# SteveMacenski/slam_toolbox

Measured on NVIDIA H100. Metric: scan matches/sec (1081-beam, +-2m/+-20deg), higher is better.
Workload: dtype u8

## Files before the change

### include/b200slam.h

```cpp
#ifndef B200SLAM_H
#define B200SLAM_H

#include <stdint.h>

#ifdef __cplusplus
extern "C" {
#endif

#define B200_OK 0
#define B200_ERR_INVALID_ARG 1
#define B200_ERR_CUDA 2
#define B200_ERR_UNSUPPORTED 3
#define B200_ERR_NOT_FOUND 4
#define B200_ERR_NUMERIC 5

const char * b200_last_error(void);
int b200_set_device(int ordinal);
int b200_device_count(void);
void b200_parallel_for(int32_t n, void (*fn)(int32_t, void *), void * ctx);
int32_t b200_host_threads(void);


typedef struct b200sm_params {
  double search_size;
// ... 51 lines not shown
                        const int32_t * pair_query, const int32_t * pair_chain, int32_t npairs,
                        int32_t do_penalize);
int b200sm_batch_run(b200sm * h);
int b200sm_batch_fetch(b200sm * h, double * response, double * mean, double * cov);
int b200sm_batch_kernel_ms(b200sm * h, float * ms);
int b200sm_batch_best(b200sm * h, int32_t * best_sum, int32_t * best_index, int32_t * tie_count);
int b200sm_batch_reduce_keys(b200sm * h, void * device_keys, int64_t id_offset);
int32_t b200sm_batch_winner_record_bytes(void);
int b200sm_batch_winner_records(b200sm * h, void * device_records, int64_t id_offset);
int b200sm_batch_winners_select(b200sm * h, const void * device_gathered, int32_t nranks, int64_t * winner_id,
                                double * response, double * mean, double * cov);
int b200sm_batch_info(b200sm * h, int32_t info[8]);
int b200sm_batch_tile_info(b200sm * h, int32_t info[8]);
int b200sm_batch_tile_layout(b200sm * h, int32_t layout[4]);
int b200sm_batch_tile_stats(b200sm * h, int32_t stats[8]);
int b200sm_batch_fetch_stats(b200sm * h, int32_t stats[4]);
int b200sm_batch_upload_timing(b200sm * h, double out[3]);
int b200sm_batch_transfer_bytes(b200sm * h, int64_t * h2d_bytes, int64_t * d2h_bytes, int32_t reset);
int b200sm_set_option(b200sm * h, const char * name, int32_t value);
int b200sm_match_timing(b200sm * h, double out[6], int32_t reset);
int64_t b200sm_launch_count(const b200sm * h);


typedef struct b200pg_opts {
  int32_t max_num_iterations;
  double function_tolerance;
  double gradient_tolerance;
  double parameter_tolerance;
  double min_relative_decrease;
  double initial_trust_region_radius;
// ... 98 lines not shown
```

### slam_toolbox_b200/api.py

```python
from __future__ import annotations

import ctypes as C
import math
import os
from dataclasses import dataclass

import numpy as np

from . import build as _build

_DP = C.POINTER(C.c_double)
_IP = C.POINTER(C.c_int32)
_lib = None

OK, ERR_INVALID_ARG, ERR_CUDA, ERR_UNSUPPORTED, ERR_NOT_FOUND, ERR_NUMERIC = range(6)


class B200Error(RuntimeError):
    def __init__(self, code: int, msg: str):
        super().__init__(f"b200slam error {code}: {msg}")
        self.code = code


class SmParams(C.Structure):
# ... 63 lines not shown
    L.b200sm_grid_copy.argtypes = [C.c_void_p, C.POINTER(C.c_uint8), C.c_int32]
    L.b200sm_match_batch.argtypes = [C.c_void_p, C.POINTER(CScan), C.c_int32, C.POINTER(CScan), C.c_int32, _IP, C.c_int32,
                                     _IP, _IP, C.c_int32, C.c_int32, C.c_int32, _DP, _DP, _DP]
    L.b200sm_batch_upload.argtypes = [C.c_void_p, C.POINTER(CScan), C.c_int32, C.POINTER(CScan), C.c_int32, _IP, C.c_int32,
                                      _IP, _IP, C.c_int32, C.c_int32]
    L.b200sm_batch_run.argtypes = [C.c_void_p]
    L.b200sm_batch_fetch.argtypes = [C.c_void_p, _DP, _DP, _DP]
    L.b200sm_batch_kernel_ms.argtypes = [C.c_void_p, C.POINTER(C.c_float)]
    L.b200sm_batch_best.argtypes = [C.c_void_p, _IP, _IP, _IP]
    L.b200sm_batch_info.argtypes = [C.c_void_p, _IP]
    L.b200sm_batch_winner_record_bytes.restype = C.c_int32
    L.b200sm_batch_winner_records.argtypes = [C.c_void_p, C.c_void_p, C.c_int64]
    L.b200sm_batch_winners_select.argtypes = [C.c_void_p, C.c_void_p, C.c_int32, C.POINTER(C.c_int64), _DP, _DP, _DP]
    L.b200sm_batch_tile_info.argtypes = [C.c_void_p, _IP]
    L.b200sm_batch_tile_stats.argtypes = [C.c_void_p, _IP]
    L.b200sm_batch_tile_layout.argtypes = [C.c_void_p, _IP]
    L.b200sm_batch_fetch_stats.argtypes = [C.c_void_p, _IP]
    L.b200sm_batch_upload_timing.argtypes = [C.c_void_p, _DP]
    L.b200sm_batch_reduce_keys.argtypes = [C.c_void_p, C.c_void_p, C.c_int64]
    L.b200sm_batch_transfer_bytes.argtypes = [C.c_void_p, C.POINTER(C.c_int64), C.POINTER(C.c_int64), C.c_int32]
    L.b200sm_set_option.argtypes = [C.c_void_p, C.c_char_p, C.c_int32]
    L.b200sm_match_timing.argtypes = [C.c_void_p, _DP, C.c_int32]
    L.b200sm_launch_count.restype = C.c_int64
    L.b200sm_launch_count.argtypes = [C.c_void_p]
    if hasattr(L, "b200pg_create"):
        L.b200pg_default_opts.argtypes = [C.POINTER(PgOpts)]
        L.b200pg_create.argtypes = [C.POINTER(PgOpts), C.POINTER(C.c_void_p)]
        L.b200pg_destroy.argtypes = [C.c_void_p]
        L.b200pg_set_stream.argtypes = [C.c_void_p, C.c_void_p]
        L.b200pg_reset.argtypes = [C.c_void_p]
# ... 244 lines not shown
    def batch_tile_info(self):
        info = np.zeros(8, dtype=np.int32)
        _check(lib().b200sm_batch_tile_info(self._h, _ip(info)))
        lay = np.zeros(4, dtype=np.int32)
        _check(lib().b200sm_batch_tile_layout(self._h, _ip(lay)))
        return dict(available=bool(info[0]), cluster=int(info[1]), chunks=int(info[2]), bands=int(info[3]), band_rows=int(info[4]),
                    refused_reason=int(info[5]), clusters=int(info[6]), smem_kb=int(info[7]), ytile_rows=int(lay[0]),
                    ytiles=int(lay[1]), xtiles=int(lay[2]), tail=bool(lay[3]))

    def batch_tile_stats(self):
        st = np.zeros(8, dtype=np.int32)
        _check(lib().b200sm_batch_tile_stats(self._h, _ip(st)))
        return dict(blocks=int(st[0]), sub_blocks=int(st[1]), max_edge_group=int(st[2]), split_groups=int(st[3]),
                    multi_entries=int(st[4]), max_multiplicity=int(st[5]), max_plain_group=int(st[6]), wrap2_entries=int(st[7]))

    def batch_upload_timing(self):
        t = np.zeros(3)
        _check(lib().b200sm_batch_upload_timing(self._h, _dp(t)))
        return dict(lookup_tables_ms=float(t[0]), kernel_tables_ms=float(t[1]), total_ms=float(t[2]))

    def batch_fetch_stats(self):
        st = np.zeros(4, dtype=np.int32)
        _check(lib().b200sm_batch_fetch_stats(self._h, _ip(st)))
        return dict(zero_pairs=int(st[0]), fallback_pairs=int(st[1]), pairs=int(st[2]))

    def transfer_bytes(self, reset: bool = False):
        a, b = C.c_int64(), C.c_int64()
        _check(lib().b200sm_batch_transfer_bytes(self._h, C.byref(a), C.byref(b), int(reset)))
        return a.value, b.value

# ... 223 lines not shown
```

### slam_toolbox_b200/csrc/sm_sweep.cu

```cuda
#include <algorithm>
#include <chrono>
#include <cmath>
#include <cstring>
#include <vector>

#include "common.cuh"
#include "sm_math.cuh"
#include "sm_types.cuh"
#include "sm_device.cuh"
#include "sm_sweep_dev.cuh"

namespace b200 {


constexpr int kFvWarps = 4;
constexpr int kFvBytesPerPoint = 17;
__global__ void __launch_bounds__(kFvWarps * 32) k_find_valid(SweepDev d)
{
  extern __shared__ __align__(16) unsigned char s_fv[];
  const int lane = threadIdx.x & 31, warp = threadIdx.x >> 5, nw = blockDim.x >> 5;
  const int item = blockIdx.x * nw + warp;
  if (item >= d.nitems) return;
  double2 * P = reinterpret_cast<double2 *>(s_fv) + (size_t)warp * d.max_n;
  unsigned char * valid = s_fv + (size_t)nw * d.max_n * sizeof(double2) + (size_t)warp * d.max_n;
// ... 1264 lines not shown
  if (!h) return B200_ERR_INVALID_ARG;
  return sweep_fetch(h, false, response, mean, cov);
  B200_GUARD_END
}

int b200sm_batch_kernel_ms(b200sm * h, float * ms)
{
  B200_GUARD_BEGIN
  if (!h || !ms || !h->sweep.ran) return B200_ERR_INVALID_ARG;
  B200_CUDA(cudaEventSynchronize(h->sweep.ev1));
  B200_CUDA(cudaEventElapsedTime(ms, h->sweep.ev0, h->sweep.ev1));
  return B200_OK;
  B200_GUARD_END
}

int b200sm_batch_best(b200sm * h, int32_t * best_sum, int32_t * best_index, int32_t * tie_count)
{
  B200_GUARD_BEGIN
  if (!h || !h->sweep.ran) return B200_ERR_INVALID_ARG;
  SweepHost & S = h->sweep;
  B200_CUDA(cudaMemcpyAsync(S.h_out.p, S.d_out.p, (size_t)S.npairs * sizeof(PairOut), cudaMemcpyDeviceToHost, h->stream));
  B200_CUDA(cudaStreamSynchronize(h->stream));
  for (int p = 0; p < S.npairs; ++p) {
    if (best_sum) best_sum[p] = S.h_out.p[p].best_sum;
    if (best_index) best_index[p] = S.h_out.p[p].tie_count > 0 ? S.h_out.p[p].ties[0] : -1;
    if (tie_count) tie_count[p] = S.h_out.p[p].tie_count;
  }
  return B200_OK;
  B200_GUARD_END
}
// ... 151 lines not shown
```

### slam_toolbox_b200/csrc/sm_tile.cu

```cuda
#include <algorithm>
#include <cmath>
#include <cstdlib>
#include <cstring>
#include <type_traits>
#include <vector>

#include "common.cuh"
#include "sm_math.cuh"
#include "sm_types.cuh"
#include "sm_device.cuh"
#include "sm_sweep_dev.cuh"

namespace b200 {

constexpr int kRowTiles = 6;
constexpr int kChunkBeams = 640;
constexpr int kMaxSingles = 63;
constexpr int kMaxPairs = 255;

__device__ __forceinline__ uint32_t smem_u32(const void * p) { return (uint32_t)__cvta_generic_to_shared(p); }
__device__ __forceinline__ void mbar_init(uint32_t bar, uint32_t count)
{
  asm volatile("mbarrier.init.shared::cta.b64 [%0], %1;" ::"r"(bar), "r"(count) : "memory");
}
// ... 81 lines not shown
    a.L2 = bL2 > a.L2 ? bL2 : a.L2;
  } else if (bL > a.L) {
    double l2 = a.L > a.L2 ? a.L : a.L2;
    l2 = bL2 > l2 ? bL2 : l2;
    a.L = bL; a.L2 = l2; a.cnt = bcnt; a.sum0 = bsum0;
    const int nb = bcnt < kMaxTies ? bcnt : kMaxTies;
    for (int t = 0; t < nb; ++t) a.ties[t] = bties[t];
  } else {
    double l2 = bL > a.L2 ? bL : a.L2;
    a.L2 = bL2 > l2 ? bL2 : l2;
  }
}

struct TileShared {
  unsigned long long bar[4];
  uint8_t kern[256];
  int ctr[2];
  double dscratch[32];
  int iscratch[32];
  TieRes chunk;
  TieRes res;
  double rankL[kTileMaxCluster], rankL2[kTileMaxCluster];
  int rankCnt[kTileMaxCluster], rankSum0[kTileMaxCluster];
  int rankTies[kTileMaxCluster][kMaxTies];
  double avg[2];
  double acc[4];
  int ok;
};

#ifdef B200_TILE_TIMERS
enum { kTmRaster, kTmDesc, kTmCorr, kTmFlush, kTmBarrier, kTmReduce, kTmPair, kTmTotal, kTmCount };
__device__ unsigned long long g_tile_timers[kTmCount];
#define TILE_TM_DECL                              \
  unsigned long long tm_acc[kTmCount] = {};       \
  long long tm_t = clock64();                     \
  const long long tm_start = tm_t;
#define TILE_TM(sec)                                                      \
  do {                                                                    \
    const long long tm_now = clock64();                                   \
    tm_acc[sec] += (unsigned long long)(tm_now - tm_t);                   \
    tm_t = tm_now;                                                        \
  } while (0)
#define TILE_TM_END                                                                 \
  do {                                                                              \
    TILE_TM(kTmPair);                                                               \
    tm_acc[kTmTotal] = (unsigned long long)(tm_t - tm_start);                       \
    if (lane == 0)                                                                  \
      for (int s = 0; s < kTmCount; ++s) atomicAdd(&g_tile_timers[s], tm_acc[s]);   \
  } while (0)
#else
#define TILE_TM_DECL
#define TILE_TM(sec) do {} while (0)
#define TILE_TM_END do {} while (0)
#endif

template <int kPitchW, bool kTail>
__global__ void __launch_bounds__(kTileThreads, 1) k_sweep_tile(SweepDev d, TileDev f)
{
  constexpr int kMain = kTail ? kRowTiles - 1 : kRowTiles;
  constexpr int kYTile = 8 * kMain;
  extern __shared__ __align__(128) unsigned char s_raw[];
  __shared__ TileShared sh;
  uint32_t * S = reinterpret_cast<uint32_t *>(s_raw);
  uint8_t * S8 = s_raw;
  int32_t * A = reinterpret_cast<int32_t *>(s_raw + f.off_A);
  double * probs = reinterpret_cast<double *>(s_raw + f.off_probs);
  int32_t * iprobs = reinterpret_cast<int32_t *>(s_raw + f.off_probs);
  const int C = f.C;
  const uint32_t rank = C > 1 ? cluster_rank() : 0u;
  const int cluster_id = blockIdx.x / C, nclusters = gridDim.x / C;
  const int nX = d.nX, nY = d.nY, nA = d.nA, P = nX * nY;
  const int half = d.ksize / 2, taps = d.ksize * d.ksize;
  const int tid = threadIdx.x, lane = tid & 31;
  const int y_l = lane >> 2, j_l = lane & 3;
  const int pitch_w = kPitchW ? kPitchW : f.pitch_w, pitchB = pitch_w * 4;
  const int sub_words = f.alloc_rows * pitch_w;
  const int nb = f.nbands;
  const uint32_t bar0 = smem_u32(&sh.bar[0]);
  const uint32_t stg0 = smem_u32(s_raw + f.off_stage);
  TILE_TM_DECL

  if (tid == 0) {
    mbar_init(bar0, 1);
    mbar_init(bar0 + 8, 1);
    mbar_init(bar0 + 16, 1);
    mbar_init(bar0 + 24, 1);
    asm volatile("fence.mbarrier_init.release.cluster;" ::: "memory");
    sh.ctr[0] = 0; sh.ctr[1] = 0;
  }
  const bool kern_smem = taps <= 256;
  if (kern_smem && tid < taps) sh.kern[tid] = d.kern[tid];
  const uint8_t * kern = kern_smem ? sh.kern : d.kern;
  __syncthreads();
  if (C > 1) { cluster_arrive(); cluster_wait(); }

  uint32_t cnt = 0;
  bool pending_wait = false;
  auto issue = [&](const TileSeq * e, uint32_t buf) {
    mbar_expect_tx(bar0 + 8 * buf, (uint32_t)e->bytes);
    bulk_g2s(stg0 + buf * (uint32_t)f.stage_bytes, f.desc + e->off, (uint32_t)e->bytes, bar0 + 8 * buf);
  };
  const uint32_t cel0 = smem_u32(s_raw + f.off_cells);
  const uint32_t cell_bytes = (uint32_t)f.cell_cap * 4u;
  auto issue_cells = [&](int pr, uint32_t buf) {
    const int it = min(d.pair_item_start[pr], max(d.nitems - 1, 0));
    mbar_expect_tx(bar0 + 16 + 8 * buf, cell_bytes);
    bulk_g2s(cel0 + buf * cell_bytes, d.cells + (size_t)it * d.max_n, cell_bytes, bar0 + 16 + 8 * buf);
  };
  if (cluster_id < d.npairs && tid == 0) {
    const int q0 = d.pair_query[cluster_id];
    issue(f.seq + f.seq_start[q0 * C + rank], 0);
    if (f.cell_cap) issue_cells(cluster_id, 0);
  }

  int iter = 0;
  for (int pair = cluster_id; pair < d.npairs; pair += nclusters, ++iter) {
    const int q = d.pair_query[pair];
    const uint32_t leader = (uint32_t)(iter % C);
    const TileSeq * seq = f.seq + f.seq_start[q * C + rank];
    const int nseq = f.seq_start[q * C + rank + 1] - f.seq_start[q * C + rank];
    const int it0 = d.pair_item_start[pair], it1 = d.pair_item_start[pair + 1];
    bool first_chunk = true;
    const int32_t * cells0 = d.cells + (size_t)it0 * d.max_n;
    const int ncell0 = it0 < it1 ? d.cell_count[it0] : 0;
    if (f.cell_cap) {
      if (tid == 0 && pair + nclusters < d.npairs) issue_cells(pair + nclusters, (uint32_t)((iter + 1) & 1));
      mbar_wait(bar0 + 16 + 8 * (iter & 1), (uint32_t)((iter >> 1) & 1));
      cells0 = reinterpret_cast<const int32_t *>(s_raw + f.off_cells + (size_t)(iter & 1) * cell_bytes);
    }
    TILE_TM(kTmPair);

    for (int si = 0; si < nseq; ++si) {
      const TileSeq e = seq[si];
      const int chunk_a0 = e.chunk * f.nAc;
      const int chunk_na = min(f.nAc, nA - chunk_a0);
      const int ph = e.stage / nb, band = e.stage - ph * nb;
      const int pp = ph & 1, pq = ph >> 1;
      const int band_r0 = band * f.band_rows;
      if (e.flags & kSeqNewChunk)
        for (int i = tid; i < chunk_na * P; i += kTileThreads) A[i] = 0;
      if (e.flags & kSeqNewStage) {
        {
          uint4 * S4 = reinterpret_cast<uint4 *>(s_raw);
          const uint4 zero = make_uint4(0u, 0u, 0u, 0u);
          for (int i = tid; i < (sub_words >> 2); i += kTileThreads) S4[i] = zero;
        }
        __syncthreads();
        const int nlev = f.nlevels;
        for (int lv = 0; lv < (nlev > 0 ? nlev : 1); ++lv) {
          const uint32_t want = nlev > 0 ? f.level[lv] : 0u;
          for (int it = it0; it < it1; ++it) {
            const int32_t * cl = it == it0 ? cells0 : d.cells + (size_t)it * d.max_n;
            const int ncell = it == it0 ? ncell0 : d.cell_count[it];
            for (int t = tid; t < ncell; t += kTileThreads) {
              const int32_t cell = cl[t];
              if (cell < 0) continue;
              const int cx = (cell & 0xFFFF) + d.roi_x - half, cy = (cell >> 16) + d.roi_y - half;
              for (int ky = (cy ^ pq) & 1; ky < d.ksize; ky += 2) {
                const int rel = ((cy + ky) >> 1) - band_r0;
                if ((unsigned)rel >= (unsigned)f.alloc_rows) continue;
                for (int kx = (cx ^ pp) & 1; kx < d.ksize; kx += 2) {
                  const uint32_t kv = kern[ky * d.ksize + kx];
                  if (nlev > 0) { if (kv == want) S8[rel * pitchB + ((cx + kx) >> 1)] = (uint8_t)kv; }
                  else if (kv) atomic_max_u8(S8 + rel * pitchB + ((cx + kx) >> 1), kv);
                }
              }
            }
          }
          if (lv + 1 < nlev) __syncthreads();
        }
      }
      if (e.flags & (kSeqNewChunk | kSeqNewStage)) __syncthreads();
      TILE_TM(kTmRaster);
      if (tid == 0) {
        const TileSeq * nxt = nullptr;
        if (si + 1 < nseq) nxt = seq + si + 1;
        else if (pair + nclusters < d.npairs) nxt = f.seq + f.seq_start[d.pair_query[pair + nclusters] * C + rank];
        if (nxt) issue(nxt, (cnt + 1) & 1);
      }
      mbar_wait(bar0 + 8 * (cnt & 1), (cnt >> 1) & 1);
      TILE_TM(kTmDesc);
      const unsigned char * stg = s_raw + f.off_stage + (size_t)(cnt & 1) * f.stage_bytes;
      const uint2 * items = reinterpret_cast<const uint2 *>(stg);
      const uint16_t * pay = reinterpret_cast<const uint16_t *>(stg + (((size_t)e.nitems * 8 + 15) & ~(size_t)15));
      for (;;) {
        int item = 0;
        if (lane == 0) item = atomicAdd(&sh.ctr[cnt & 1], 1);
        item = __shfl_sync(0xffffffffu, item, 0);
        if (item >= e.nitems) break;
        const uint2 rec = items[item];
        const int b0 = (int)(rec.x & 0xFFFFu);
        int b = b0;
        const int pe = b0 + (int)((rec.x >> 16) & 0x3FFu), se = pe + 2 * (int)(rec.x >> 26);
// ... 417 lines not shown
    case 132: return (const void *)k_sweep_tile<132, kTail>;
    default: return (const void *)k_sweep_tile<0, kTail>;
  }
}
static const void * tile_kernel_for(int pitch_w, bool tail)
{
  return tail ? tile_kernel_for_layout<true>(pitch_w) : tile_kernel_for_layout<false>(pitch_w);
}

static int env_int(const char * name, int dflt)
{
  const char * v = std::getenv(name);
  return (v && *v) ? std::atoi(v) : dflt;
}

static inline bool d_max_n_ok(int max_n) { return max_n > 0 && (max_n & 3) == 0 && max_n <= 4096; }

static inline int floor_div(int a, int b) { return a >= 0 ? a / b : -((-a + b - 1) / b); }

static void spread_rows(std::vector<uint16_t>::iterator b, std::vector<uint16_t>::iterator e)
{
  const size_t L = (size_t)(e - b), R = (L + 7) / 8;
  if (L < 9) return;
  const std::vector<uint16_t> src(b, e);
  size_t o = 0;
  for (size_t j = 0; j < R; ++j)
    for (size_t y = 0; y < 8; ++y)
      if (y * R + j < L) b[o++] = src[y * R + j];
}

static bool build_block_items(const std::vector<int32_t> & tbl, const std::vector<int> & nedge, int na, int xtiles, int ytiles,
                              std::vector<uint2> & out)
// ... 84 lines not shown
    const int one_angle = 8 * xtiles * ytiles * (4 + std::max(n - 1, 0) / kChunkBeams) + 2 * n + 4 * 12 + 6 + 10;
    int stage = 16 + nAc * 52 + (nAc * n * 2 * 3) / 8 + 64 * nAc;
    stage = std::max(stage, one_angle + 64);
    stage = (stage + 127) & ~127;
    const int s_avail = budget - a_bytes - probs_bytes - 2 * stage;
    if (s_avail <= 0) continue;
    int rows_avail = s_avail / (pitch_w * 4);
    if ((long)rows_avail * pitch_w > 65535) rows_avail = 65535 / pitch_w;
    int B = rows_avail - halo;
    if (B < 8) continue;
    B = std::min(B, base_rows);
    const int nbv = (base_rows + B - 1) / B;
    B = (base_rows + nbv - 1) / nbv;
    const double loads = tail ? 5.0 * ytiles + 0.25 : 6.0 * ytiles;
    const long w_angle = (long)((double)n * xtiles * loads * 32 * 2.3 / kTileThreads) + 4L * nbv * (4L * xtiles * ytiles * 100 / 32);
    const long w_raster = 4 * (700 + 3L * std::min(B + halo, rows_valid + halo - nY) * pitch_w / kTileThreads);
    const long cost = (long)((V + Cc - 1) / Cc) * (nbv * w_raster + nAc * w_angle);
    if (bestCost < 0 || cost < bestCost) { bestCost = cost; bestV = V; bestNb = nbv; bestB = B; bestStage = stage; }
  }
  if (bestCost < 0) return bail(4);
  const int V = bestV, nbands = bestNb, B = bestB, nAc = (nA + V - 1) / V, stage_bytes = bestStage;
  const int C = std::min(Cc, V);
  int alloc_rows = std::min(B + halo, rows_valid + halo - nY);
  alloc_rows = std::max(alloc_rows, 1);
  const size_t s_bytes = ((size_t)alloc_rows * pitch_w * 4 + 15) & ~(size_t)15;
  const size_t a_bytes = ((size_t)nAc * P * 4 + 15) & ~(size_t)15;
  T.C = C; T.V = V; T.nAc = nAc; T.nbands = nbands; T.band_rows = B; T.alloc_rows = alloc_rows; T.pitch_w = pitch_w;
  T.xtiles = xtiles; T.ytiles = ytiles; T.tail = tail ? 1 : 0; T.stage_bytes = stage_bytes;
  T.int_ties = int_ties;
  {
    std::vector<uint8_t> lv(g.kernel.begin(), g.kernel.end());
    std::sort(lv.begin(), lv.end());
    lv.erase(std::unique(lv.begin(), lv.end()), lv.end());
    if (!lv.empty() && lv[0] == 0) lv.erase(lv.begin());
    T.nlevels = (!lv.empty() && lv.size() <= 4) ? (int)lv.size() : 0;
    for (int i = 0; i < 4; ++i) T.level[i] = i < T.nlevels ? lv[i] : 0;
  }
  T.off_A = s_bytes; T.off_probs = s_bytes + a_bytes; T.off_stage = (T.off_probs + probs_bytes + 127) & ~(size_t)127;
  T.off_cells = T.off_stage + 2 * (size_t)stage_bytes;
  int cell_cap = d_max_n_ok(S.max_n) ? S.max_n : 0;
  if (T.off_cells + 2 * (size_t)cell_cap * 4 + sizeof(TileShared) + 64 > 227 * 1024) cell_cap = 0;
  T.cell_cap = cell_cap;
  size_t smem = T.off_cells + 2 * (size_t)cell_cap * 4;
  const size_t overrun = (size_t)std::max(ytile_rows * ytiles - nY + 1, 1) * pitch_w * 4;
  if (smem - s_bytes < overrun) smem = s_bytes + overrun;
  if (smem + sizeof(TileShared) + 64 > 227 * 1024) return bail(5);

  const int nstage = 4 * nbands;
  std::vector<uint8_t> blob;
  std::vector<TileSeq> seq;
  std::vector<int32_t> seq_start((size_t)nq * C + 1, 0);
  std::vector<int32_t> edge, edge_start((size_t)nq * nA * nstage * 4 + 1, 0);
  std::vector<int32_t> wrap2, wrap2_start((size_t)nq * nA * nstage + 1, 0);
  std::vector<int32_t> slow, slow_start((size_t)nq * (nA + 1), 0);
  int n_fast = 0, n_edge = 0;
  std::vector<std::vector<uint16_t>> grp((size_t)nA * nstage * 4);
  std::vector<std::vector<int32_t>> egrp((size_t)nA * nstage * 4), wgrp((size_t)nA * nstage);
  blob.reserve((size_t)nq * nA * n * 2 + 4096);
// ... 201 lines not shown
    sweep_stage_h2d(dst.p, src.data(), src.size() * sizeof(TT), st);
  };
  up(S.d_tile_desc, blob);
  up(S.d_tile_seq, seq);
  up(S.d_tile_seq_start, seq_start);
  up(S.d_tile_edge, edge);
  up(S.d_tile_edge_start, edge_start);
  up(S.d_tile_wrap2, wrap2);
  up(S.d_tile_wrap2_start, wrap2_start);
  up(S.d_tile_slow, slow);
  up(S.d_tile_slow_start, slow_start);
  T.desc = S.d_tile_desc.p; T.seq = S.d_tile_seq.p; T.seq_start = S.d_tile_seq_start.p;
  T.edge = S.d_tile_edge.p; T.edge_start = S.d_tile_edge_start.p;
  T.wrap2 = S.d_tile_wrap2.p; T.wrap2_start = S.d_tile_wrap2_start.p;
  T.slow = S.d_tile_slow.p; T.slow_start = S.d_tile_slow_start.p;
  T.enabled = 1;
  S.tile_smem = smem;

  const void * kfn = tile_kernel_for(pitch_w, T.tail != 0);
  B200_CUDA(cudaFuncSetAttribute(kfn, cudaFuncAttributeMaxDynamicSharedMemorySize, (int)smem));
  int max_clusters = sms / C;
  {
    cudaLaunchConfig_t cfg{};
    cfg.gridDim = dim3((unsigned)(C * std::max(1, sms / C)));
    cfg.blockDim = dim3(kTileThreads);
    cfg.dynamicSmemBytes = smem;
    cudaLaunchAttribute at[1];
    at[0].id = cudaLaunchAttributeClusterDimension;
    at[0].val.clusterDim.x = (unsigned)C; at[0].val.clusterDim.y = 1; at[0].val.clusterDim.z = 1;
    cfg.attrs = at; cfg.numAttrs = 1;
    int nc = 0;
    if (cudaOccupancyMaxActiveClusters(&nc, kfn, &cfg) == cudaSuccess && nc > 0) max_clusters = nc;
    else (void)cudaGetLastError();
  }
  const int clusters = std::max(1, std::min(S.npairs, max_clusters));
  S.tile_grid = clusters * C;
  S.tile_info[0] = 1; S.tile_info[1] = C; S.tile_info[2] = V; S.tile_info[3] = nbands; S.tile_info[4] = B; S.tile_info[5] = 0;
  S.tile_info[6] = clusters; S.tile_info[7] = (int32_t)(smem / 1024);
  S.tile_layout[0] = ytile_rows; S.tile_layout[1] = ytiles; S.tile_layout[2] = xtiles; S.tile_layout[3] = tail ? 1 : 0;
  S.fast_info[1] = n_fast; S.fast_info[2] = n_edge; S.fast_info[3] = (int32_t)slow.size() - 1;
  return true;
}

void launch_sweep_tile(b200sm * h, SweepHost & S, cudaStream_t st)
{
  (void)h;
  cudaLaunchConfig_t cfg{};
  cfg.gridDim = dim3((unsigned)S.tile_grid);
  cfg.blockDim = dim3(kTileThreads);
  cfg.dynamicSmemBytes = S.tile_smem;
  cfg.stream = st;
  cudaLaunchAttribute at[1];
  at[0].id = cudaLaunchAttributeClusterDimension;
  at[0].val.clusterDim.x = (unsigned)S.tile.C; at[0].val.clusterDim.y = 1; at[0].val.clusterDim.z = 1;
  cfg.attrs = at; cfg.numAttrs = 1;
  const void * kfn = tile_kernel_for(S.tile.pitch_w, S.tile.tail != 0);
  B200_CUDA(cudaFuncSetAttribute(kfn, cudaFuncAttributeMaxDynamicSharedMemorySize, (int)S.tile_smem));
  void * args[] = {(void *)&S.dev, (void *)&S.tile};
  B200_CUDA(cudaLaunchKernelExC(&cfg, kfn, args));
}

}

#ifdef B200_TILE_TIMERS
extern "C" int b200_tile_timers(unsigned long long * out, int reset)
{
  using namespace b200;
  if (cudaDeviceSynchronize() != cudaSuccess) return -1;
  if (out && cudaMemcpyFromSymbol(out, g_tile_timers, sizeof(g_tile_timers)) != cudaSuccess) return -1;
  if (reset) {
    const unsigned long long zero[kTmCount] = {};
    if (cudaMemcpyToSymbol(g_tile_timers, zero, sizeof(zero)) != cudaSuccess) return -1;
  }
  return kTmCount;
}
#endif
```

### slam_toolbox_b200/csrc/sm_types.cuh

```cuda
#pragma once
#include <cstdint>
#include <functional>
#include <utility>
#include <vector>

#include "common.cuh"
#include "sm_math.cuh"

namespace b200 {

constexpr int kMaxTies = 24;
constexpr int kSweepThreads = 512;
constexpr int32_t kDevInvalid = -(1 << 30);

struct GridGeom {
  int width = 0, height = 0, stride = 0;
  int roi_x = 0, roi_y = 0, roi_w = 0, roi_h = 0;
  int data_size = 0;
  int ksize = 0;
  bool order_dependent = false;
  double scale = 0.0;
  double off_x = 0.0, off_y = 0.0;
  std::vector<uint8_t> kernel;
};
// ... 104 lines not shown
  int16_t nitems;
  uint32_t flags;
};
constexpr int kItemMaxXTiles = 64, kItemMaxYTiles = 256;
constexpr uint32_t kSeqNewChunk = 1, kSeqNewStage = 2, kSeqEndChunk = 4, kSeqHasWrap = 16;
struct TileDev {
  int enabled;
  int C, V, nAc;
  int nbands, band_rows, alloc_rows, pitch_w;
  int xtiles, ytiles;
  int tail;
  int stage_bytes;
  int nlevels;
  uint32_t level[4];
  int int_ties;
  size_t off_A, off_probs, off_stage, off_cells;
  int cell_cap;
  const uint8_t * desc;
  const TileSeq * seq;
  const int32_t * seq_start;
  const int32_t * edge;
  const int32_t * edge_start;
  const int32_t * wrap2;
  const int32_t * wrap2_start;
  const int32_t * slow;
  const int32_t * slow_start;
};

struct FineDev {
  int P, nA;
  const int32_t * offsets;
  const int32_t * posidx;
// ... 13 lines not shown
  DevBuf<double> d_qgeom, d_center, d_qd, d_angpen, d_points, d_ws_probs;
  DevBuf<uint8_t> d_ws_grid, d_kernel, d_win_flag;
  DevBuf<uint16_t> d_fast_beams, d_fast_mult;
  DevBuf<int32_t> d_fast_cls, d_fast_slow, d_fast_slow_start, d_fast_wrap2, d_fast_wrap2_start, d_fast_edge, d_fast_edge_start;
  FastDev fast{};
  size_t fast_smem = 0;
  TileDev tile{};
  size_t tile_smem = 0;
  int tile_grid = 0;
  int32_t tile_info[8] = {0, 0, 0, 0, 0, 0, 0, 0};
  int32_t tile_stats[8] = {0, 0, 0, 0, 0, 0, 0, 0};
  int32_t tile_layout[4] = {0, 0, 0, 0};
  DevBuf<uint8_t> d_tile_desc;
  DevBuf<TileSeq> d_tile_seq;
  DevBuf<int32_t> d_tile_seq_start, d_tile_edge, d_tile_edge_start, d_tile_wrap2, d_tile_wrap2_start, d_tile_slow, d_tile_slow_start;
  int32_t fast_info[5] = {0, 0, 0, 0, 0};
  int fast_blocks = 0;
  DevBuf<PairOut> d_out;
  PinBuf<PairOut> h_out;
  PinBuf<uint8_t> arena;
  size_t arena_used = 0;
  PinBuf<int32_t> h_i;
  PinBuf<double> h_d;
  SweepDev dev{};
  cudaEvent_t ev0 = nullptr, ev1 = nullptr;
  int64_t h2d_bytes = 0, d2h_bytes = 0;
  int zero_pairs = 0, fallback_pairs = 0;
  double upload_ms[3] = {0, 0, 0};
  std::vector<char> zero_done, zero_exp_done;
  std::vector<double> zero_mean, zero_cov, zero_exp_mean, zero_exp_cov;
// ... 33 lines not shown
  }
};

namespace b200 {
double do_match(b200sm * h, const b200_scan * query, const b200_scan * base, int nbase, bool pen, bool refine,
                double mean[3], double cov[9]);
int32_t device_offset(int32_t off, int data_size);
void set_grid_offset(GridGeom & g, const b200_scan * query);
double normalize_angle_difference(double minuend, double subtrahend);
}

namespace b200 {
bool build_tile_tables(b200sm * h, SweepHost & S, cudaStream_t st);
void sweep_stage_h2d(void * dst, const void * src, size_t bytes, cudaStream_t s);
void launch_sweep_tile(b200sm * h, SweepHost & S, cudaStream_t st);
double host_epilogue(const b200sm_params & prm, const GridGeom & geom, int probs_side, const CorrPlan & pl,
                     const int32_t * sums, bool do_penalize, double mean[3], double cov[9],
                     const std::function<bool(int, int, int32_t *)> * extra_cell = nullptr);
}
```

Baseline: 471,100.

## Precompute sparse rasterized grid words in a separate kernel and replay them in tile sweep

Moves per-stage smear rasterization out of the tiled correlation kernel into a new pre-pass kernel. The pre-pass builds each pair's four parity-phase images in shared memory and compacts their nonzero 32-bit words into (index, value) lists with per-band ranges. The sweep kernel now bulk-loads those word slices asynchronously, double-buffered, and scatters them into the stage image. It clears only the previously written words instead of zeroing the whole sub-image. This removes repeated atomic rasterization from every band and angle chunk, at the cost of an extra launch, a large device buffer, and pair-range batching. The tile cost model is also retuned to match.

```diff
diff --git a/include/b200slam.h b/include/b200slam.h
--- a/include/b200slam.h
+++ b/include/b200slam.h
@@ -89,6 +89,7 @@
 int b200sm_batch_tile_info(b200sm * h, int32_t info[8]);
 int b200sm_batch_tile_layout(b200sm * h, int32_t layout[4]);
 int b200sm_batch_tile_stats(b200sm * h, int32_t stats[8]);
+int b200sm_batch_raster_words(b200sm * h, int32_t pair, int32_t info[8], int32_t * band, uint32_t * words, int32_t cap);
 int b200sm_batch_fetch_stats(b200sm * h, int32_t stats[4]);
 int b200sm_batch_upload_timing(b200sm * h, double out[3]);
 int b200sm_batch_transfer_bytes(b200sm * h, int64_t * h2d_bytes, int64_t * d2h_bytes, int32_t reset);
diff --git a/slam_toolbox_b200/api.py b/slam_toolbox_b200/api.py
--- a/slam_toolbox_b200/api.py
+++ b/slam_toolbox_b200/api.py
@@ -101,6 +101,7 @@
     L.b200sm_batch_winners_select.argtypes = [C.c_void_p, C.c_void_p, C.c_int32, C.POINTER(C.c_int64), _DP, _DP, _DP]
     L.b200sm_batch_tile_info.argtypes = [C.c_void_p, _IP]
     L.b200sm_batch_tile_stats.argtypes = [C.c_void_p, _IP]
+    L.b200sm_batch_raster_words.argtypes = [C.c_void_p, C.c_int32, _IP, _IP, C.POINTER(C.c_uint32), C.c_int32]
     L.b200sm_batch_tile_layout.argtypes = [C.c_void_p, _IP]
     L.b200sm_batch_fetch_stats.argtypes = [C.c_void_p, _IP]
     L.b200sm_batch_upload_timing.argtypes = [C.c_void_p, _DP]
@@ -375,6 +376,18 @@
         return dict(blocks=int(st[0]), sub_blocks=int(st[1]), max_edge_group=int(st[2]), split_groups=int(st[3]),
                     multi_entries=int(st[4]), max_multiplicity=int(st[5]), max_plain_group=int(st[6]), wrap2_entries=int(st[7]))
 
+    def batch_raster_words(self, pair: int, cap: int = 1 << 20):
+        info = np.zeros(8, dtype=np.int32)
+        band = np.zeros(4 * max(self.batch_tile_info()["bands"], 1) * 2, dtype=np.int32)
+        words = np.zeros(2 * cap, dtype=np.uint32)
+        _check(lib().b200sm_batch_raster_words(self._h, int(pair), _ip(info), _ip(band), words.ctypes.data_as(C.POINTER(C.c_uint32)), cap))
+        nb = int(info[1])
+        counts = [int(c) for c in info[4:8]]
+        starts = np.concatenate([[0], np.cumsum(counts)])
+        return dict(pitch_w=int(info[0]), nbands=nb, band_rows=int(info[2]), alloc_rows=int(info[3]),
+                    phases=[words[2 * starts[p]:2 * starts[p + 1]].reshape(-1, 2).copy() for p in range(4)],
+                    bands=[band[2 * p * nb:2 * (p + 1) * nb].reshape(nb, 2).copy() for p in range(4)])
+
     def batch_upload_timing(self):
         t = np.zeros(3)
         _check(lib().b200sm_batch_upload_timing(self._h, _dp(t)))
diff --git a/slam_toolbox_b200/csrc/sm_sweep.cu b/slam_toolbox_b200/csrc/sm_sweep.cu
--- a/slam_toolbox_b200/csrc/sm_sweep.cu
+++ b/slam_toolbox_b200/csrc/sm_sweep.cu
@@ -1302,6 +1302,17 @@
   B200_GUARD_END
 }
 
+int b200sm_batch_raster_words(b200sm * h, int32_t pair, int32_t info[8], int32_t * band, uint32_t * words, int32_t cap)
+{
+  B200_GUARD_BEGIN
+  if (!h || !info || !band || !words || cap < 0) return B200_ERR_INVALID_ARG;
+  const int r = raster_words_of_pair(h, pair, info, band, words, cap);
+  if (r == -1) { set_last_error("batch_raster_words: no tiled sweep has run, or pair out of range"); return B200_ERR_INVALID_ARG; }
+  if (r == -2) { set_last_error("batch_raster_words: words buffer too small"); return B200_ERR_INVALID_ARG; }
+  return B200_OK;
+  B200_GUARD_END
+}
+
 int b200sm_batch_best(b200sm * h, int32_t * best_sum, int32_t * best_index, int32_t * tie_count)
 {
   B200_GUARD_BEGIN
diff --git a/slam_toolbox_b200/csrc/sm_tile.cu b/slam_toolbox_b200/csrc/sm_tile.cu
--- a/slam_toolbox_b200/csrc/sm_tile.cu
+++ b/slam_toolbox_b200/csrc/sm_tile.cu
@@ -119,7 +119,7 @@
 
 struct TileShared {
   unsigned long long bar[4];
-  uint8_t kern[256];
+  int wslice[2][2];
   int ctr[2];
   double dscratch[32];
   int iscratch[32];
@@ -134,7 +134,7 @@
 };
 
 #ifdef B200_TILE_TIMERS
-enum { kTmRaster, kTmDesc, kTmCorr, kTmFlush, kTmBarrier, kTmReduce, kTmPair, kTmTotal, kTmCount };
+enum { kTmReplay, kTmDesc, kTmCorr, kTmFlush, kTmBarrier, kTmReduce, kTmPair, kTmTotal, kTmCount };
 __device__ unsigned long long g_tile_timers[kTmCount];
 #define TILE_TM_DECL                              \
   unsigned long long tm_acc[kTmCount] = {};       \
@@ -159,6 +159,89 @@
 #define TILE_TM_END do {} while (0)
 #endif
 
+constexpr int kRwThreads = 1024;
+constexpr int kRwImageBytes = 100 * 1024;
+
+__global__ void __launch_bounds__(kRwThreads, 2) k_raster_words(SweepDev d, TileDev f)
+{
+  extern __shared__ __align__(16) unsigned char s_img[];
+  __shared__ uint8_t s_kern[256];
+  __shared__ int s_scan[32];
+  const int pair = f.pair0 + (int)(blockIdx.x >> 2), ph = (int)(blockIdx.x & 3);
+  const int pp = ph & 1, pq = ph >> 1;
+  const int tid = threadIdx.x;
+  const int half = d.ksize / 2, taps = d.ksize * d.ksize;
+  const int pitch_w = f.pitch_w, pitchB = 4 * pitch_w, nb = f.nbands, B = f.band_rows;
+  const int rows_total = (nb - 1) * B + f.alloc_rows;
+  const bool kern_smem = taps <= 256;
+  if (kern_smem && tid < taps) s_kern[tid] = d.kern[tid];
+  const uint8_t * kern = kern_smem ? s_kern : d.kern;
+  const int it0 = d.pair_item_start[pair], it1 = d.pair_item_start[pair + 1];
+  const int base = f.rw_base[pair * 4 + ph];
+  uint2 * out = f.rw + base;
+  int32_t * band = f.rw_band + (size_t)(pair * 4 + ph) * nb * 2;
+  const int nlev = f.nlevels;
+  int written = 0;
+  for (int r0 = 0; r0 < rows_total; r0 += f.rw_piece_rows) {
+    const int nrows = min(f.rw_piece_rows, rows_total - r0), words = nrows * pitch_w;
+    for (int i = tid; i < (words >> 2); i += kRwThreads) reinterpret_cast<uint4 *>(s_img)[i] = make_uint4(0u, 0u, 0u, 0u);
+    __syncthreads();
+    for (int lv = 0; lv < (nlev > 0 ? nlev : 1); ++lv) {
+      const uint32_t want = nlev > 0 ? f.level[lv] : 0u;
+      for (int it = it0; it < it1; ++it) {
+        const int32_t * cl = d.cells + (size_t)it * d.max_n;
+        const int ncell = d.cell_count[it];
+        for (int t = tid; t < ncell; t += kRwThreads) {
+          const int32_t cell = cl[t];
+          if (cell < 0) continue;
+          const int cx = (cell & 0xFFFF) + d.roi_x - half, cy = (cell >> 16) + d.roi_y - half;
+          for (int ky = (cy ^ pq) & 1; ky < d.ksize; ky += 2) {
+            const int rel = ((cy + ky) >> 1) - r0;
+            if ((unsigned)rel >= (unsigned)nrows) continue;
+            for (int kx = (cx ^ pp) & 1; kx < d.ksize; kx += 2) {
+              const int col = (cx + kx) >> 1;
+              if ((unsigned)col >= (unsigned)pitchB) continue;
+              const uint32_t kv = kern[ky * d.ksize + kx];
+              if (nlev > 0) { if (kv == want) s_img[rel * pitchB + col] = (uint8_t)kv; }
+              else if (kv) atomic_max_u8(s_img + rel * pitchB + col, kv);
+            }
+          }
+        }
+      }
+      __syncthreads();
+    }
+    const uint4 * img4 = reinterpret_cast<const uint4 *>(s_img);
+    const int groups = words >> 2, row_groups = pitch_w >> 2;
+    const int per = (groups + kRwThreads - 1) / kRwThreads;
+    const int g0 = min(groups, tid * per), g1 = min(groups, g0 + per);
+    int c = 0;
+    for (int gi = g0; gi < g1; ++gi) {
+      const uint4 v = img4[gi];
+      c += (v.x != 0u) + (v.y != 0u) + (v.z != 0u) + (v.w != 0u);
+    }
+    int total = 0;
+    int k = written + block_exclusive_scan(c, s_scan, total);
+    int row = r0 + g0 / row_groups, col = g0 - (g0 / row_groups) * row_groups;
+    for (int gi = g0; gi < g1; ++gi) {
+      if (col == 0) {
+        if (row % B == 0 && row / B < nb) band[2 * (row / B)] = base + k;
+        const int e = row - f.alloc_rows;
+        if (e >= 0 && e % B == 0 && e / B < nb) band[2 * (e / B) + 1] = base + k;
+      }
+      const uint4 v = img4[gi];
+      const uint32_t w = (uint32_t)(r0 * pitch_w + 4 * gi);
+      if (v.x) out[k++] = make_uint2(w, v.x);
+      if (v.y) out[k++] = make_uint2(w + 1, v.y);
+      if (v.z) out[k++] = make_uint2(w + 2, v.z);
+      if (v.w) out[k++] = make_uint2(w + 3, v.w);
+      if (++col == row_groups) { col = 0; ++row; }
+    }
+    written += total;
+    __syncthreads();
+  }
+  if (tid == 0) band[2 * (nb - 1) + 1] = base + written;
+}
+
 template <int kPitchW, bool kTail>
 __global__ void __launch_bounds__(kTileThreads, 1) k_sweep_tile(SweepDev d, TileDev f)
 {
@@ -175,7 +258,6 @@
   const uint32_t rank = C > 1 ? cluster_rank() : 0u;
   const int cluster_id = blockIdx.x / C, nclusters = gridDim.x / C;
   const int nX = d.nX, nY = d.nY, nA = d.nA, P = nX * nY;
-  const int half = d.ksize / 2, taps = d.ksize * d.ksize;
   const int tid = threadIdx.x, lane = tid & 31;
   const int y_l = lane >> 2, j_l = lane & 3;
   const int pitch_w = kPitchW ? kPitchW : f.pitch_w, pitchB = pitch_w * 4;
@@ -193,46 +275,52 @@
     asm volatile("fence.mbarrier_init.release.cluster;" ::: "memory");
     sh.ctr[0] = 0; sh.ctr[1] = 0;
   }
-  const bool kern_smem = taps <= 256;
-  if (kern_smem && tid < taps) sh.kern[tid] = d.kern[tid];
-  const uint8_t * kern = kern_smem ? sh.kern : d.kern;
   __syncthreads();
   if (C > 1) { cluster_arrive(); cluster_wait(); }
 
   uint32_t cnt = 0;
+  uint32_t scnt = 0;
   bool pending_wait = false;
   auto issue = [&](const TileSeq * e, uint32_t buf) {
     mbar_expect_tx(bar0 + 8 * buf, (uint32_t)e->bytes);
     bulk_g2s(stg0 + buf * (uint32_t)f.stage_bytes, f.desc + e->off, (uint32_t)e->bytes, bar0 + 8 * buf);
   };
-  const uint32_t cel0 = smem_u32(s_raw + f.off_cells);
-  const uint32_t cell_bytes = (uint32_t)f.cell_cap * 4u;
-  auto issue_cells = [&](int pr, uint32_t buf) {
-    const int it = min(d.pair_item_start[pr], max(d.nitems - 1, 0));
-    mbar_expect_tx(bar0 + 16 + 8 * buf, cell_bytes);
-    bulk_g2s(cel0 + buf * cell_bytes, d.cells + (size_t)it * d.max_n, cell_bytes, bar0 + 16 + 8 * buf);
+  const uint32_t wst0 = smem_u32(s_raw + f.off_words);
+  const uint32_t words_bytes = ((uint32_t)f.words_cap + 2u) * 8u;
+  auto issue_words = [&](int pr, int stg, uint32_t buf) {
+    const int32_t * sl = f.rw_band + ((size_t)pr * 4 * f.nbands + stg) * 2;
+    const int b = sl[0], e = sl[1];
+    sh.wslice[buf][0] = b; sh.wslice[buf][1] = e;
+    const int a0 = b & ~1, n = ((e + 1) & ~1) - a0;
+    const uint32_t wbar = bar0 + 16 + 8 * buf;
+    if (e > b && n <= f.words_cap) {
+      asm volatile("fence.proxy.async.shared::cta;" ::: "memory");
+      mbar_expect_tx(wbar, (uint32_t)n * 8u);
+      bulk_g2s(wst0 + buf * words_bytes, f.rw + a0, (uint32_t)n * 8u, wbar);
+    } else {
+      mbar_expect_tx(wbar, 0u);
+    }
   };
-  if (cluster_id < d.npairs && tid == 0) {
-    const int q0 = d.pair_query[cluster_id];
-    issue(f.seq + f.seq_start[q0 * C + rank], 0);
-    if (f.cell_cap) issue_cells(cluster_id, 0);
+  auto words_src = [&](uint32_t buf) -> const uint2 * {
+    const int b = sh.wslice[buf][0], e = sh.wslice[buf][1];
+    if (e > b && ((e + 1) & ~1) - (b & ~1) <= f.words_cap)
+      return reinterpret_cast<const uint2 *>(s_raw + f.off_words + (size_t)buf * words_bytes) + (b & 1);
+    return f.rw + b;
+  };
+  int prev_shift = 0;
+  if (f.pair0 + cluster_id < f.pair1 && tid == 0) {
+    const TileSeq * s0 = f.seq + f.seq_start[d.pair_query[f.pair0 + cluster_id] * C + rank];
+    issue(s0, 0);
+    issue_words(f.pair0 + cluster_id, s0->stage, 0);
   }
 
   int iter = 0;
-  for (int pair = cluster_id; pair < d.npairs; pair += nclusters, ++iter) {
+  for (int pair = f.pair0 + cluster_id; pair < f.pair1; pair += nclusters, ++iter) {
     const int q = d.pair_query[pair];
     const uint32_t leader = (uint32_t)(iter % C);
     const TileSeq * seq = f.seq + f.seq_start[q * C + rank];
     const int nseq = f.seq_start[q * C + rank + 1] - f.seq_start[q * C + rank];
-    const int it0 = d.pair_item_start[pair], it1 = d.pair_item_start[pair + 1];
     bool first_chunk = true;
-    const int32_t * cells0 = d.cells + (size_t)it0 * d.max_n;
-    const int ncell0 = it0 < it1 ? d.cell_count[it0] : 0;
-    if (f.cell_cap) {
-      if (tid == 0 && pair + nclusters < d.npairs) issue_cells(pair + nclusters, (uint32_t)((iter + 1) & 1));
-      mbar_wait(bar0 + 16 + 8 * (iter & 1), (uint32_t)((iter >> 1) & 1));
-      cells0 = reinterpret_cast<const int32_t *>(s_raw + f.off_cells + (size_t)(iter & 1) * cell_bytes);
-    }
     TILE_TM(kTmPair);
 
     for (int si = 0; si < nseq; ++si) {
@@ -245,43 +333,42 @@
       if (e.flags & kSeqNewChunk)
         for (int i = tid; i < chunk_na * P; i += kTileThreads) A[i] = 0;
       if (e.flags & kSeqNewStage) {
-        {
+        if (e.flags & kSeqNewChunk && first_chunk) {
           uint4 * S4 = reinterpret_cast<uint4 *>(s_raw);
           const uint4 zero = make_uint4(0u, 0u, 0u, 0u);
           for (int i = tid; i < (sub_words >> 2); i += kTileThreads) S4[i] = zero;
-        }
+        } else {
+          const uint32_t pb = (scnt + 1) & 1;
+          const int wb = sh.wslice[pb][0], nw = sh.wslice[pb][1] - wb;
+          const uint2 * src = words_src(pb);
+          for (int i = tid; i < nw; i += kTileThreads) S[(int)src[i].x - prev_shift] = 0u;
+        }
+        mbar_wait(bar0 + 16 + 8 * (scnt & 1), (scnt >> 1) & 1);
         __syncthreads();
-        const int nlev = f.nlevels;
-        for (int lv = 0; lv < (nlev > 0 ? nlev : 1); ++lv) {
-          const uint32_t want = nlev > 0 ? f.level[lv] : 0u;
-          for (int it = it0; it < it1; ++it) {
-            const int32_t * cl = it == it0 ? cells0 : d.cells + (size_t)it * d.max_n;
-            const int ncell = it == it0 ? ncell0 : d.cell_count[it];
-            for (int t = tid; t < ncell; t += kTileThreads) {
-              const int32_t cell = cl[t];
-              if (cell < 0) continue;
-              const int cx = (cell & 0xFFFF) + d.roi_x - half, cy = (cell >> 16) + d.roi_y - half;
-              for (int ky = (cy ^ pq) & 1; ky < d.ksize; ky += 2) {
-                const int rel = ((cy + ky) >> 1) - band_r0;
-                if ((unsigned)rel >= (unsigned)f.alloc_rows) continue;
-                for (int kx = (cx ^ pp) & 1; kx < d.ksize; kx += 2) {
-                  const uint32_t kv = kern[ky * d.ksize + kx];
-                  if (nlev > 0) { if (kv == want) S8[rel * pitchB + ((cx + kx) >> 1)] = (uint8_t)kv; }
-                  else if (kv) atomic_max_u8(S8 + rel * pitchB + ((cx + kx) >> 1), kv);
-                }
-              }
-            }
-          }
-          if (lv + 1 < nlev) __syncthreads();
-        }
+        const int nw = sh.wslice[scnt & 1][1] - sh.wslice[scnt & 1][0];
+        const uint2 * src = words_src(scnt & 1);
+        const int shift = band_r0 * pitch_w;
+        for (int i = tid; i < nw; i += kTileThreads) {
+          const uint2 w = src[i];
+          S[(int)w.x - shift] = w.y;
+        }
+        prev_shift = shift;
+        ++scnt;
       }
       if (e.flags & (kSeqNewChunk | kSeqNewStage)) __syncthreads();
-      TILE_TM(kTmRaster);
+      TILE_TM(kTmReplay);
       if (tid == 0) {
         const TileSeq * nxt = nullptr;
         if (si + 1 < nseq) nxt = seq + si + 1;
-        else if (pair + nclusters < d.npairs) nxt = f.seq + f.seq_start[d.pair_query[pair + nclusters] * C + rank];
+        else if (pair + nclusters < f.pair1) nxt = f.seq + f.seq_start[d.pair_query[pair + nclusters] * C + rank];
         if (nxt) issue(nxt, (cnt + 1) & 1);
+        if (e.flags & kSeqNewStage) {
+          int sj = si + 1;
+          while (sj < nseq && !(seq[sj].flags & kSeqNewStage)) ++sj;
+          if (sj < nseq) issue_words(pair, seq[sj].stage, scnt & 1);
+          else if (pair + nclusters < f.pair1)
+            issue_words(pair + nclusters, f.seq[f.seq_start[d.pair_query[pair + nclusters] * C + rank]].stage, scnt & 1);
+        }
       }
       mbar_wait(bar0 + 8 * (cnt & 1), (cnt >> 1) & 1);
       TILE_TM(kTmDesc);
@@ -729,8 +816,6 @@
   return (v && *v) ? std::atoi(v) : dflt;
 }
 
-static inline bool d_max_n_ok(int max_n) { return max_n > 0 && (max_n & 3) == 0 && max_n <= 4096; }
-
 static inline int floor_div(int a, int b) { return a >= 0 ? a / b : -((-a + b - 1) / b); }
 
 static void spread_rows(std::vector<uint16_t>::iterator b, std::vector<uint16_t>::iterator e)
@@ -845,8 +930,9 @@
     B = (base_rows + nbv - 1) / nbv;
     const double loads = tail ? 5.0 * ytiles + 0.25 : 6.0 * ytiles;
     const long w_angle = (long)((double)n * xtiles * loads * 32 * 2.3 / kTileThreads) + 4L * nbv * (4L * xtiles * ytiles * 100 / 32);
-    const long w_raster = 4 * (700 + 3L * std::min(B + halo, rows_valid + halo - nY) * pitch_w / kTileThreads);
-    const long cost = (long)((V + Cc - 1) / Cc) * (nbv * w_raster + nAc * w_angle);
+    const long w_raster = 4 * (150 + 3L * std::min(B + halo, rows_valid + halo - nY) * pitch_w / kTileThreads);
+    long cost = 0;
+    for (int v = 0; v < V; v += Cc) cost += nbv * w_raster + (long)std::min(nAc, nA - v * nAc) * w_angle;
     if (bestCost < 0 || cost < bestCost) { bestCost = cost; bestV = V; bestNb = nbv; bestB = B; bestStage = stage; }
   }
   if (bestCost < 0) return bail(4);
@@ -868,11 +954,12 @@
     for (int i = 0; i < 4; ++i) T.level[i] = i < T.nlevels ? lv[i] : 0;
   }
   T.off_A = s_bytes; T.off_probs = s_bytes + a_bytes; T.off_stage = (T.off_probs + probs_bytes + 127) & ~(size_t)127;
-  T.off_cells = T.off_stage + 2 * (size_t)stage_bytes;
-  int cell_cap = d_max_n_ok(S.max_n) ? S.max_n : 0;
-  if (T.off_cells + 2 * (size_t)cell_cap * 4 + sizeof(TileShared) + 64 > 227 * 1024) cell_cap = 0;
-  T.cell_cap = cell_cap;
-  size_t smem = T.off_cells + 2 * (size_t)cell_cap * 4;
+  T.off_words = T.off_stage + 2 * (size_t)stage_bytes;
+  const long words_room = (long)(227 * 1024) - (long)T.off_words - (long)sizeof(TileShared) - 1024;
+  int words_cap = (int)std::min<long>(words_room / 16 - 2, 8192) & ~1;
+  if (words_cap < 64) words_cap = 0;
+  T.words_cap = words_cap;
+  size_t smem = T.off_words + (words_cap ? 2 * ((size_t)words_cap + 2) * 8 : 0);
   const size_t overrun = (size_t)std::max(ytile_rows * ytiles - nY + 1, 1) * pitch_w * 4;
   if (smem - s_bytes < overrun) smem = s_bytes + overrun;
   if (smem + sizeof(TileShared) + 64 > 227 * 1024) return bail(5);
@@ -1104,6 +1191,34 @@
   T.edge = S.d_tile_edge.p; T.edge_start = S.d_tile_edge_start.p;
   T.wrap2 = S.d_tile_wrap2.p; T.wrap2_start = S.d_tile_wrap2_start.p;
   T.slow = S.d_tile_slow.p; T.slow_start = S.d_tile_slow_start.p;
+
+  {
+    const long rows_total = (long)(nbands - 1) * B + alloc_rows;
+    const long sub_words_total = rows_total * pitch_w;
+    const long hk = (g.ksize + 1) / 2;
+    const long cap_entries = std::min<long>(std::max(1, env_int("B200_RASTER_WORDS_CAP_MB", 2048)) * (1024L * 1024 / 8), 1L << 30);
+    std::vector<int32_t> rw_base((size_t)S.npairs * 4);
+    S.rw_ranges.assign(1, 0);
+    long used = 0, max_used = 0;
+    for (int p = 0; p < S.npairs; ++p) {
+      const int c = S.pair_chain[p];
+      const long cells = (long)(S.chain_start[c + 1] - S.chain_start[c]) * S.max_n;
+      const long per = (std::min(sub_words_total, hk * hk * cells) + 1) & ~1L;
+      if (used > 0 && used + 4 * per > cap_entries) { S.rw_ranges.push_back(p); used = 0; }
+      for (int ph = 0; ph < 4; ++ph) rw_base[(size_t)p * 4 + ph] = (int32_t)(used + ph * per);
+      used += 4 * per;
+      max_used = std::max(max_used, used);
+    }
+    S.rw_ranges.push_back(S.npairs);
+    S.d_rw.reserve((size_t)max_used + 2);
+    S.d_rw_band.reserve(std::max<size_t>((size_t)S.npairs * 4 * nbands * 2, 1));
+    up(S.d_rw_base, rw_base);
+    T.rw = S.d_rw.p; T.rw_base = S.d_rw_base.p; T.rw_band = S.d_rw_band.p;
+    const long max_rows = std::max<long>(1, kRwImageBytes / (pitch_w * 4)), pieces = (rows_total + max_rows - 1) / max_rows;
+    T.rw_piece_rows = (int)((rows_total + pieces - 1) / pieces);
+    S.rw_smem = (size_t)T.rw_piece_rows * pitch_w * 4;
+    B200_CUDA(cudaFuncSetAttribute(k_raster_words, cudaFuncAttributeMaxDynamicSharedMemorySize, (int)S.rw_smem));
+  }
   T.enabled = 1;
   S.tile_smem = smem;
 
@@ -1132,22 +1247,82 @@
   return true;
 }
 
+#ifdef B200_TILE_TIMERS
+static double g_rw_ms = 0.0;
+#endif
+
+static void launch_raster_words(const SweepHost & S, const TileDev & T, cudaStream_t st)
+{
+#ifdef B200_TILE_TIMERS
+  cudaEvent_t e0, e1;
+  B200_CUDA(cudaEventCreate(&e0)); B200_CUDA(cudaEventCreate(&e1));
+  B200_CUDA(cudaEventRecord(e0, st));
+#endif
+  k_raster_words<<<(unsigned)(T.pair1 - T.pair0) * 4, kRwThreads, S.rw_smem, st>>>(S.dev, T);
+  B200_CUDA(cudaGetLastError());
+#ifdef B200_TILE_TIMERS
+  B200_CUDA(cudaEventRecord(e1, st));
+  B200_CUDA(cudaEventSynchronize(e1));
+  float ms = 0.f;
+  B200_CUDA(cudaEventElapsedTime(&ms, e0, e1));
+  g_rw_ms += ms;
+  cudaEventDestroy(e0); cudaEventDestroy(e1);
+#endif
+}
+
 void launch_sweep_tile(b200sm * h, SweepHost & S, cudaStream_t st)
 {
-  (void)h;
-  cudaLaunchConfig_t cfg{};
-  cfg.gridDim = dim3((unsigned)S.tile_grid);
-  cfg.blockDim = dim3(kTileThreads);
-  cfg.dynamicSmemBytes = S.tile_smem;
-  cfg.stream = st;
-  cudaLaunchAttribute at[1];
-  at[0].id = cudaLaunchAttributeClusterDimension;
-  at[0].val.clusterDim.x = (unsigned)S.tile.C; at[0].val.clusterDim.y = 1; at[0].val.clusterDim.z = 1;
-  cfg.attrs = at; cfg.numAttrs = 1;
   const void * kfn = tile_kernel_for(S.tile.pitch_w, S.tile.tail != 0);
   B200_CUDA(cudaFuncSetAttribute(kfn, cudaFuncAttributeMaxDynamicSharedMemorySize, (int)S.tile_smem));
-  void * args[] = {(void *)&S.dev, (void *)&S.tile};
-  B200_CUDA(cudaLaunchKernelExC(&cfg, kfn, args));
+  B200_CUDA(cudaFuncSetAttribute(k_raster_words, cudaFuncAttributeMaxDynamicSharedMemorySize, (int)S.rw_smem));
+  for (size_t k = 0; k + 1 < S.rw_ranges.size(); ++k) {
+    TileDev T = S.tile;
+    T.pair0 = S.rw_ranges[k]; T.pair1 = S.rw_ranges[k + 1];
+    if (T.pair1 <= T.pair0) continue;
+    launch_raster_words(S, T, st);
+    cudaLaunchConfig_t cfg{};
+    cfg.gridDim = dim3((unsigned)std::min(S.tile_grid, S.tile.C * (T.pair1 - T.pair0)));
+    cfg.blockDim = dim3(kTileThreads);
+    cfg.dynamicSmemBytes = S.tile_smem;
+    cfg.stream = st;
+    cudaLaunchAttribute at[1];
+    at[0].id = cudaLaunchAttributeClusterDimension;
+    at[0].val.clusterDim.x = (unsigned)S.tile.C; at[0].val.clusterDim.y = 1; at[0].val.clusterDim.z = 1;
+    cfg.attrs = at; cfg.numAttrs = 1;
+    void * args[] = {(void *)&S.dev, (void *)&T};
+    B200_CUDA(cudaLaunchKernelExC(&cfg, kfn, args));
+    if (k > 0) h->launches += 2;
+  }
+  h->launches += 1;
+}
+
+int raster_words_of_pair(b200sm * h, int pair, int32_t * info, int32_t * band, uint32_t * words, int cap)
+{
+  SweepHost & S = h->sweep;
+  if (!S.ran || !S.tile.enabled || pair < 0 || pair >= S.npairs) return -1;
+  const TileDev & T0 = S.tile;
+  const int nb = T0.nbands;
+  TileDev T = T0;
+  T.pair0 = pair; T.pair1 = pair + 1;
+  cudaStream_t st = h->stream;
+  launch_raster_words(S, T, st);
+  std::vector<int32_t> bt((size_t)4 * nb * 2), base(4);
+  B200_CUDA(cudaMemcpyAsync(bt.data(), T.rw_band + (size_t)pair * 4 * nb * 2, bt.size() * 4, cudaMemcpyDeviceToHost, st));
+  B200_CUDA(cudaMemcpyAsync(base.data(), T.rw_base + (size_t)pair * 4, 16, cudaMemcpyDeviceToHost, st));
+  B200_CUDA(cudaStreamSynchronize(st));
+  info[0] = T.pitch_w; info[1] = nb; info[2] = T.band_rows; info[3] = T.alloc_rows;
+  int total = 0;
+  for (int ph = 0; ph < 4; ++ph) {
+    const int cnt = bt[(size_t)(ph * nb + nb - 1) * 2 + 1] - base[ph];
+    info[4 + ph] = cnt;
+    for (int b = 0; b < nb; ++b)
+      for (int k = 0; k < 2; ++k) band[(ph * nb + b) * 2 + k] = bt[(size_t)(ph * nb + b) * 2 + k] - base[ph];
+    if (total + cnt > cap) return -2;
+    if (cnt > 0)
+      B200_CUDA(cudaMemcpy(words + 2 * (size_t)total, T.rw + base[ph], (size_t)cnt * 8, cudaMemcpyDeviceToHost));
+    total += cnt;
+  }
+  return total;
 }
 
 }
@@ -1164,4 +1339,11 @@
   }
   return kTmCount;
 }
+
+extern "C" double b200_raster_words_ms(int reset)
+{
+  const double v = b200::g_rw_ms;
+  if (reset) b200::g_rw_ms = 0.0;
+  return v;
+}
 #endif
diff --git a/slam_toolbox_b200/csrc/sm_types.cuh b/slam_toolbox_b200/csrc/sm_types.cuh
--- a/slam_toolbox_b200/csrc/sm_types.cuh
+++ b/slam_toolbox_b200/csrc/sm_types.cuh
@@ -142,8 +142,13 @@
   int nlevels;
   uint32_t level[4];
   int int_ties;
-  size_t off_A, off_probs, off_stage, off_cells;
-  int cell_cap;
+  size_t off_A, off_probs, off_stage, off_words;
+  int words_cap;
+  int pair0, pair1;
+  int rw_piece_rows;
+  uint2 * rw;
+  const int32_t * rw_base;
+  int32_t * rw_band;
   const uint8_t * desc;
   const TileSeq * seq;
   const int32_t * seq_start;
@@ -187,6 +192,10 @@
   DevBuf<uint8_t> d_tile_desc;
   DevBuf<TileSeq> d_tile_seq;
   DevBuf<int32_t> d_tile_seq_start, d_tile_edge, d_tile_edge_start, d_tile_wrap2, d_tile_wrap2_start, d_tile_slow, d_tile_slow_start;
+  DevBuf<uint2> d_rw;
+  DevBuf<int32_t> d_rw_base, d_rw_band;
+  std::vector<int32_t> rw_ranges;
+  size_t rw_smem = 0;
   int32_t fast_info[5] = {0, 0, 0, 0, 0};
   int fast_blocks = 0;
   DevBuf<PairOut> d_out;
@@ -250,6 +259,7 @@
 bool build_tile_tables(b200sm * h, SweepHost & S, cudaStream_t st);
 void sweep_stage_h2d(void * dst, const void * src, size_t bytes, cudaStream_t s);
 void launch_sweep_tile(b200sm * h, SweepHost & S, cudaStream_t st);
+int raster_words_of_pair(b200sm * h, int pair, int32_t * info, int32_t * band, uint32_t * words, int cap);
 double host_epilogue(const b200sm_params & prm, const GridGeom & geom, int probs_side, const CorrPlan & pl,
                      const int32_t * sums, bool do_penalize, double mean[3], double cov[9],
                      const std::function<bool(int, int, int32_t *)> * extra_cell = nullptr);
```

New measurement: 471,900, median of 6. No clear change (+0.2%).
